# matthewygf/Tiresias

Measured on AMD Instinct MI355X. Metric: avg JCT + makespan on NSDI'19 Microsoft trace, 8×MI355X cluster, lower is better.
Workload: dtype bf16

## Files before the change

### csrc/bindings/ops.cpp

```cpp
#include <array>
#include <ATen/ATen.h>
#include <c10/hip/HIPStream.h>
#include <torch/library.h>

#include <functional>
#include <map>
#include <mutex>
#include <sstream>
#include <tuple>
#include <vector>

#include "tam/kernels.h"
#include "tam/launch.h"
#include "tam/gemm8p.h"

using at::Tensor;
using c10::optional;

namespace {

hipStream_t cur_stream(const Tensor& t) {
  return c10::hip::getCurrentHIPStream(t.device().index()).stream();
}

// ... 903 lines not shown
void avgpool_backward_op(const Tensor& dy, const Tensor& dx) {
  check_bf16(dy, "dy"); check_bf16(dx, "dx"); check_contig(dx, "dx");
  tam::avgpool_backward(bp(dy), bpm(dx), (int)dx.size(0), (int)(dx.size(1) * dx.size(2)),
                        (int)dx.size(3), cur_stream(dy));
}

void softmax_xent_op(const Tensor& logits, const Tensor& labels, const optional<Tensor>& dlogits,
                     const Tensor& loss_rows, double smoothing, double grad_scale,
                     int64_t ignore_index, int64_t tm_b) {
  check_bf16(logits, "logits"); check_contig(logits, "logits");
  TORCH_CHECK(labels.scalar_type() == at::kLong && labels.is_cuda() && labels.is_contiguous(),
              "tam.xent: labels contiguous int64 GPU");
  check_f32(loss_rows, "loss_rows");
  const int64_t V = logits.size(-1), rows = logits.numel() / V;
  TORCH_CHECK(labels.numel() == rows && loss_rows.numel() == rows, "tam.xent: row count");
  TORCH_CHECK(tm_b <= 0 || rows % tm_b == 0, "tam.xent: tm_b must divide the rows");
  tam::softmax_xent(bp(logits), labels.data_ptr<int64_t>(), opt_ptr<tam::bf16_t>(dlogits),
                    loss_rows.data_ptr<float>(), rows, (int)V, (float)smoothing, (float)grad_scale,
                    ignore_index, cur_stream(logits), tm_b);
}

void embedding_forward_op(const Tensor& table, const Tensor& ids, const Tensor& out, double scale, int64_t tm_b,
                          const optional<Tensor>& pos) {
  check_bf16(table, "table"); check_bf16(out, "out"); check_contig(table, "table");
  TORCH_CHECK(ids.scalar_type() == at::kLong && ids.is_contiguous(), "tam.embedding: ids");
  const int64_t D = table.size(1);
  TORCH_CHECK(D % 8 == 0, "tam.embedding: D % 8");
  TORCH_CHECK(out.numel() == ids.numel() * D, "tam.embedding: out size");
  TORCH_CHECK(tm_b <= 0 || ids.numel() % tm_b == 0, "tam.embedding: tm_b must divide the ids");
  const tam::bf16_t* pp = nullptr;
  int64_t prow = 0;
  if (pos.has_value() && pos->defined()) {
    check_bf16(*pos, "pos"); check_contig(*pos, "pos");
    TORCH_CHECK(pos->dim() == 2 && pos->size(1) == D, "tam.embedding: pos must be [S][D]");
    prow = pos->size(0);
    TORCH_CHECK(prow > 0 && (tm_b > 0 ? ids.numel() / tm_b == prow : ids.numel() % prow == 0),
                "tam.embedding: pos rows must equal the sequence length");
    pp = bp(*pos);
  }
  tam::embedding_forward(bp(table), ids.data_ptr<int64_t>(), bpm(out), ids.numel(), (int)D,
                         (float)scale, cur_stream(table), table.size(0), tm_b, pp, prow);
}
void embedding_backward_op(const Tensor& dout, const Tensor& ids, const Tensor& gtable, double scale, int64_t tm_b) {
  check_bf16(dout, "dout"); check_f32(gtable, "gtable"); check_contig(dout, "dout");
  TORCH_CHECK(ids.scalar_type() == at::kLong && ids.is_contiguous() && gtable.dim() == 2 &&
                  dout.numel() == ids.numel() * gtable.size(1), "tam.embedding_backward: shapes");
  TORCH_CHECK(tm_b <= 0 || ids.numel() % tm_b == 0, "tam.embedding_backward: tm_b must divide the ids");
  tam::embedding_backward(bp(dout), ids.data_ptr<int64_t>(), gtable.data_ptr<float>(), ids.numel(),
                          (int)gtable.size(1), (float)scale, cur_stream(dout), gtable.size(0), tm_b);
}

void conv_dma_policy_op(int64_t p) { tam::conv_dma_policy((int)p); }
void conv_halo_policy_op(int64_t p) { tam::conv_halo_policy((int)p); }
void colsum_policy_op(int64_t p) { tam::colsum_policy((int)p); }
void attn_short_policy_op(int64_t p) { tam::attn_short_policy((int)p); }
void conv_wgrad_c64_policy_op(int64_t p) { tam::conv_wgrad_c64_policy((int)p); }
void conv_wgrad_order_op(int64_t p) { tam::conv_wgrad_order((int)p); }
void conv_stem_policy_op(int64_t p) { tam::conv_stem_policy((int)p); }
void conv_wgrad_slab_policy_op(int64_t p) { tam::conv_wgrad_slab_policy((int)p); }
void conv_wgrad_force_op(int64_t bm, int64_t bn, int64_t splits, int64_t noatomic) {
  tam::conv_wgrad_force((int)bm, (int)bn, (int)splits, (int)noatomic);
}
int g_dma_policy = 1;
TAM_KNOB(g_dma_policy)
void gemm_dma_policy_op(int64_t p, int64_t cfg) {
  g_dma_policy = (int)p;
  tam::gemm_dma_policy(p == 2 ? 1 : 0, (int)cfg);
}

void gemm8p_policy_op(int64_t mode, int64_t tile) { tam::gemm8p_policy((int)mode, (int)tile); }
void gemm_pw_policy_op(int64_t on) { tam::gemm_pw_policy((int)on); }
void conv_pw_gemm_policy_op(int64_t mode, int64_t tile) { tam::conv_pw_gemm_policy((int)mode, (int)tile); }

std::string policy_names_op() {
  std::string out;
  for (const auto& k : tam::knob_registry()) {
    if (!out.empty()) out += ",";
    out += k.name;
  }
  return out;
}
std::vector<int64_t> policy_state_op() {
  std::vector<int64_t> v;
  for (const auto& k : tam::knob_registry()) v.push_back(*k.p);
  return v;
}
void policy_load_op(std::vector<int64_t> v) {
  auto& reg = tam::knob_registry();
  TORCH_CHECK(v.size() == reg.size(), "policy_load: ", v.size(), " values for ", reg.size(), " knobs");
  for (size_t i = 0; i < reg.size(); ++i) *reg[i].p = (int)v[i];
}
void gemm8p_group_op(int64_t g) { tam::gemm8p_group((int)g); }
void gemm8p_slab_force_op(int64_t sp) { tam::gemm8p_slab_force((int)sp); }
void gemm8p_sk_force_op(int64_t on) { g_sk_force = on != 0; }
void conv_split_policy_op(int64_t p) { tam::conv_split_policy((int)p); }
void optim_grid_op(int64_t b) { tam::optim_grid((int)b); }
void optim_variant_op(int64_t v) { tam::optim_variant((int)v); }
void gemm_skinny_policy_op(int64_t on, int64_t sp, int64_t nst) {
  tam::gemm_skinny_policy((int)on, (int)sp, (int)nst);
}

void gemm_force_op(int64_t cfg, int64_t splits) {
  tam::gemm_force((int)cfg, (int)splits);
  g_forced = cfg >= 0 || splits >= 1;
}

// ... 403 lines not shown
  m.def("conv_fwd(Tensor x, Tensor w, Tensor(a!) y, int stride, int pad, int dil, Tensor? bias, bool relu, Tensor(b!)? stats=None) -> int", &conv_fwd_op);
  m.def("conv_dgrad(Tensor dy, Tensor w, Tensor(a!) wt, Tensor(b!) dx, int stride, int pad, int dil, Tensor? mask) -> ()", &conv_dgrad_op);
  m.def("conv_weight_t_batch(Tensor[] w, Tensor(a!)[] wt) -> ()", &conv_weight_t_batch_op);
  m.def("gemm_wgrad_grouped(Tensor[] dy, Tensor[] x, Tensor(a!)[] dw, Tensor(b!)[] db, int[]? modes=None) -> ()", &gemm_wgrad_grouped_op);
  m.def("gemm_wgrad_grouped_ok(int M, int N, int K) -> bool", &gemm_wgrad_grouped_ok_op);
  m.def("gemm_grouped_tile(int tile) -> ()", &gemm_grouped_tile_op);
  m.def("conv_dgrad_pre(Tensor dy, Tensor w, Tensor wt, Tensor(a!) dx, int stride, int pad, int dil, Tensor? mask, Tensor(b!)? stats=None, Tensor? bnx=None, Tensor? bnmean=None, Tensor? bnrstd=None) -> int", &conv_dgrad_pre_op);
  m.def("conv_wgrad(Tensor dy, Tensor x, Tensor(a!) dw, int stride, int pad, int dil, int mode, Tensor(b!)? dbias=None, bool patch=True) -> ()", &conv_wgrad_op);
  m.def("conv_wgrad_deferred(Tensor dy, Tensor x, Tensor(a!) dw, int stride, int pad, int dil, int mode, Tensor(b!)? dbias, bool patch) -> (Tensor, int)", &conv_wgrad_deferred_op);
  m.def("wgrad_slab_reduce_many(Tensor[] slabs, int[] sp, Tensor(a!)[] dw, int[] mode) -> ()", &wgrad_slab_reduce_many_op);
  m.def("bn_forward(Tensor x, Tensor? res, Tensor(a!) y, Tensor gamma, Tensor beta, Tensor(b!)? run_mean, Tensor(c!)? run_var, Tensor(d!) save_mean, Tensor(e!) save_rstd, float eps, float momentum, bool relu, Tensor(f!)? sums=None, bool sums_ready=False, Tensor(g!)? ymask=None) -> ()", &bn_forward_op);
  m.def("bn_backward(Tensor dy, Tensor? y, Tensor x, Tensor mean, Tensor rstd, Tensor gamma, Tensor(a!) dx, Tensor(b!)? dres, Tensor(c!)? dgamma, Tensor(d!)? dbeta, bool relu, Tensor? addend=None, Tensor(e!)? sums=None, bool sums_ready=False, Tensor? ymask=None) -> ()", &bn_backward_op);
  m.def("ln_forward(Tensor x, Tensor g, Tensor b, Tensor(a!) y, Tensor(b!) mean, Tensor(c!) rstd, float eps, Tensor? addend=None, Tensor(d!)? sum_out=None, Tensor? drop_rec=None, int drop_site=0, int drop_thr=0, float drop_scale=1.0) -> ()", &ln_forward_op);
  m.def("ln_backward(Tensor dy, Tensor x, Tensor g, Tensor mean, Tensor rstd, Tensor(a!) dx, Tensor(b!) dg, Tensor(c!) db, Tensor? addend=None, Tensor(d!)? dr=None, Tensor? drop_rec=None, int drop_site=0, int drop_thr=0, float drop_scale=1.0) -> ()", &ln_backward_op);
  m.def("ln_backward_split(Tensor dy, Tensor x, Tensor g, Tensor mean, Tensor rstd, Tensor(a!) dx, Tensor(b!) ws, Tensor? addend=None, Tensor(c!)? dr=None, Tensor? drop_rec=None, int drop_site=0, int drop_thr=0, float drop_scale=1.0) -> int", &ln_backward_split_op);
  m.def("dropout_apply(Tensor x, Tensor(a!) y, Tensor rec, int site, int thr, float scale) -> ()", &dropout_apply_op);
  m.def("dropout_advance(Tensor(a!) rec) -> ()", &dropout_advance_op);
  m.def("col_reduce_acc(Tensor part, int nblk, int W, Tensor(a!) out0, Tensor(b!) out1, int split) -> ()", &col_reduce_acc_op);
  m.def("col_reduce_acc_batch(Tensor[] parts, int[] nblk, Tensor(a!)[] out0, Tensor(b!)[] out1) -> ()", &col_reduce_acc_batch_op);
  m.def("maxpool_forward(Tensor x, Tensor(a!) y, Tensor(b!) idx, int R, int S, int stride, int pad) -> ()", &maxpool_forward_op);
  m.def("maxpool_backward(Tensor dy, Tensor idx, Tensor(a!) dx, int R, int S, int stride, int pad) -> ()", &maxpool_backward_op);
  m.def("maxpool_k3s2_policy(int policy) -> ()", &maxpool_k3s2_policy_op);
  m.def("avgpool_forward(Tensor x, Tensor(a!) y) -> ()", &avgpool_forward_op);
  m.def("avgpool_backward(Tensor dy, Tensor(a!) dx) -> ()", &avgpool_backward_op);
  m.def("softmax_xent(Tensor logits, Tensor labels, Tensor(a!)? dlogits, Tensor(b!) loss_rows, float smoothing, float grad_scale, int ignore_index, int tm_b=0) -> ()", &softmax_xent_op);
  m.def("embedding_forward(Tensor table, Tensor ids, Tensor(a!) out, float scale, int tm_b=0, Tensor? pos=None) -> ()", &embedding_forward_op);
  m.def("embedding_backward(Tensor dout, Tensor ids, Tensor(a!) gtable, float scale, int tm_b=0) -> ()", &embedding_backward_op);
  m.def("sum_scale(Tensor x, Tensor(a!) out, float scale) -> ()", &sum_scale_op);
  m.def("rows_sum(Tensor[] outs, Tensor[] ins, int[] n_in) -> ()", &rows_sum_op);
  m.def("zero_(Tensor(a!) t) -> ()", &zero_op);
  m.def("colsum(Tensor x, Tensor(a!) out) -> ()", &colsum_op);
  m.def("gemm_force(int cfg, int splits) -> ()", &gemm_force_op);
  m.def("gemm8p_policy(int mode, int tile) -> ()", &gemm8p_policy_op);
  m.def("gemm_pw_policy(int on) -> ()", &gemm_pw_policy_op);
  m.def("conv_pw_gemm_policy(int mode, int tile) -> ()", &conv_pw_gemm_policy_op);
  m.def("policy_names() -> str", &policy_names_op);
  m.def("policy_state() -> int[]", &policy_state_op);
  m.def("policy_load(int[] v) -> ()", &policy_load_op);
  m.def("gemm8p_group(int g) -> ()", &gemm8p_group_op);
  m.def("gemm8p_slab_force(int sp) -> ()", &gemm8p_slab_force_op);
  m.def("gemm_skinny_policy(int on, int force_splits, int nst) -> ()", &gemm_skinny_policy_op);
  m.def("gemm8p_sk_force(int on) -> ()", &gemm8p_sk_force_op);
  m.def("conv_split_policy(int p) -> ()", &conv_split_policy_op);
  m.def("optim_variant(int v) -> ()", &optim_variant_op);
  m.def("optim_grid(int blocks) -> ()", &optim_grid_op);
  m.def("gemm_lib_policy(int policy) -> ()", &gemm_lib_policy_op);
  m.def("conv_dma_policy(int policy) -> ()", &conv_dma_policy_op);
  m.def("conv_wgrad_force(int bm, int bn, int splits, int noatomic=0) -> ()", &conv_wgrad_force_op);
  m.def("conv_wgrad_c64_policy(int policy) -> ()", &conv_wgrad_c64_policy_op);
  m.def("conv_wgrad_order(int flat) -> ()", &conv_wgrad_order_op);
  m.def("conv_stem_policy(int policy) -> ()", &conv_stem_policy_op);
  m.def("conv_wgrad_slab_policy(int policy) -> ()", &conv_wgrad_slab_policy_op);
  m.def("conv_halo_policy(int policy) -> ()", &conv_halo_policy_op);
  m.def("colsum_policy(int policy) -> ()", &colsum_policy_op);
  m.def("attn_short_policy(int policy) -> ()", &attn_short_policy_op);
  m.def("gemm_dma_policy(int policy, int cfg) -> ()", &gemm_dma_policy_op);
  m.def("gemm_routes() -> str", &gemm_routes_op);
  m.def("relu_backward(Tensor dy, Tensor y, Tensor(a!) dx) -> ()", &relu_backward_op);
  m.def("add(Tensor a, Tensor b, Tensor(a!) y) -> ()", &add_op);
  m.def("cast_f32_bf16(Tensor x, Tensor(a!) y) -> ()", &cast_op);
  m.def("sgd_step(Tensor(a!) w, Tensor(b!) g, Tensor(c!) mom, Tensor(d!) wb, float lr, float momentum, float wd, float gscale, bool nesterov, bool zero_grad, Tensor? guard=None, int zero_from=0, int wd_until=-1, Tensor? clip=None) -> ()", &sgd_op);
  m.def("adam_step(Tensor(a!) w, Tensor(b!) g, Tensor(c!) m, Tensor(d!) v, Tensor(e!) wb, float lr, float b1, float b2, float eps, float wd, int step, float gscale, bool zero_grad, Tensor? guard=None, int zero_from=0, int wd_until=-1, Tensor? clip=None) -> ()", &adam_op);
  m.def("sgd_step_bf16s(Tensor(a!) w, Tensor(b!) g, Tensor(c!) mom, Tensor(d!) wb, float lr, float momentum, float wd, float gscale, bool nesterov, bool zero_grad, int seed, int step, int base=0, Tensor? guard=None, int zero_from=0, int wd_until=-1, Tensor? clip=None) -> ()", &sgd_bf16s_op);
  m.def("adam_step_bf16s(Tensor(a!) w, Tensor(b!) g, Tensor(c!) m, Tensor(d!) v, Tensor(e!) wb, float lr, float b1, float b2, float eps, float wd, int step, float gscale, bool zero_grad, int seed, int base=0, Tensor? guard=None, int zero_from=0, int wd_until=-1, Tensor? clip=None) -> ()", &adam_bf16s_op);
  m.def("grad_sumsq(Tensor g, Tensor(a!) partials) -> ()", &grad_sumsq_op);
  m.def("grad_clip_finalize(Tensor partials, float max_norm, float gscale, Tensor(a!) clip) -> ()", &grad_clip_finalize_op);
  m.def("grad_sumsq_blocks(int n) -> int", &grad_sumsq_blocks_op);
  m.def("lars_step(Tensor(a!) w, Tensor(b!) g, Tensor(c!) mom, Tensor(d!) wb, float lr, float momentum, float wd, float eta, float gscale, Tensor tiles, Tensor seg_first, Tensor(e!) partials, Tensor(f!) ratios, Tensor? guard=None, int zero_from=0, int wd_until=-1, Tensor? clip=None) -> ()", &lars_op);
  m.def("lamb_step(Tensor(a!) w, Tensor(b!) g, Tensor(c!) m, Tensor(d!) v, Tensor(e!) wb, float lr, float b1, float b2, float eps, float wd, int step, float eta, float gscale, Tensor tiles, Tensor seg_first, Tensor(f!) partials, Tensor(g!) ratios, Tensor? guard=None, int zero_from=0, int wd_until=-1, Tensor? clip=None) -> ()", &lamb_op);
  m.def("trust_tile() -> int", &trust_tile_op);
  m.def("lstm_guard_step(Tensor(a!) err) -> ()", &lstm_guard_step_op);
  m.def("attn_forward(Tensor q, Tensor k, Tensor v, Tensor(a!) o, Tensor(b!) lse, bool causal, float scale, Tensor? kv_len, Tensor? drop_rec=None, int drop_site=0, int drop_thr=0, float drop_scale=1.0) -> ()", &attn_forward_op);
  m.def("attn_backward(Tensor q, Tensor k, Tensor v, Tensor o, Tensor dout, Tensor lse, Tensor(a!) dq, Tensor(b!) dk, Tensor(c!) dv, Tensor(d!) dq_acc, Tensor(e!) delta, bool causal, float scale, Tensor? kv_len, Tensor? drop_rec=None, int drop_site=0, int drop_thr=0, float drop_scale=1.0) -> ()", &attn_backward_op);
  m.def("lstm_step_forward(Tensor gx, Tensor w_hh, Tensor? h_prev, Tensor? c_prev, Tensor(a!) c_out, Tensor(b!) h_out, Tensor(c!) act) -> ()", &lstm_step_fwd_op);
  m.def("lstm_seq_forward(Tensor gx, Tensor w_hh, Tensor(a!) hs, Tensor(b!) cs, Tensor(c!) act, bool reverse, Tensor(d!) sync, Tensor(e!)? job_err=None, int grids=-1, int reserved_cus=0, bool zeroed=False) -> bool", &lstm_seq_fwd_op);
  m.def("lstm_seq_backward(Tensor act, Tensor cs, Tensor dH, Tensor w_hh, Tensor(a!) dG, bool reverse, Tensor(b!) sync, Tensor(c!)? job_err=None, int grids=-1, int reserved_cus=0, bool zeroed=False) -> bool", &lstm_seq_bwd_op);
  m.def("lstm_seq_policy(int ch) -> ()", &lstm_seq_policy_op);
  m.def("lstm_seq_shards(int ns) -> ()", &lstm_seq_shards_op);
  m.def("gemm_routes_load(str text) -> int", &gemm_routes_load_op);
  m.def("lstm_seq_residency(int grids, int reserved_cus) -> ()", &lstm_seq_residency_op);
  m.def("lstm_persist_timeouts(bool reset) -> int", &lstm_persist_timeouts_op);
  m.def("lstm_seq_spin_limit(int polls) -> ()", &lstm_seq_spin_limit_op);
  m.def("lstm_cell_forward(Tensor gates, Tensor? c_prev, Tensor(a!) c_out, Tensor(b!) h_out, Tensor(c!)? h_f32, Tensor(d!) act) -> ()", &lstm_fwd_op);
  m.def("lstm_cell_backward(Tensor act, Tensor? c_prev, Tensor? dh, Tensor? dc_next, Tensor(a!)? dgates, Tensor(b!)? dc_prev, Tensor(c!)? dgates_bf16) -> ()", &lstm_bwd_op);
}
```

### csrc/include/tam/conv_dma.h

```cpp
#pragma once
#include <cstdlib>
#include "tam/igemm.h"
#include "tam/slab.h"

namespace tam {

typedef __attribute__((address_space(3))) void cd_lds_void_t;

static __device__ __attribute__((aligned(256))) bf16_t g_cd_zero[128];

struct CDArgs {
  const bf16_t* src;
  const bf16_t* wgt;
  int M, Ng, Kd;
  int Hs, Ws, Cs;
  int P, Q;
  int stride, base_h, base_w;
  long ldb;
  int ntaps;
  int tap_dh[9], tap_dw[9], tap_kcol[9];
  int omap, oH, oW, osh, osw, ooh, oow;
  FastDiv fq, fp, fct;
};

// ... 121 lines not shown
    }
    if (stats) {
#pragma unroll
      for (int o = CPR; o < 64; o <<= 1)
#pragma unroll
        for (int e = 0; e < 8; ++e) {
          ssum[e] += __shfl_xor(ssum[e], o, 64);
          ssq[e] += __shfl_xor(ssq[e], o, 64);
        }
      float* red = (float*)(smem + W * 32 * LDW * 2);
      if (lane < CPR) {
#pragma unroll
        for (int e = 0; e < 8; ++e) {
          red[wid * 2 * WCOLS + lane * 8 + e] = ssum[e];
          red[wid * 2 * WCOLS + WCOLS + lane * 8 + e] = ssq[e];
        }
      }
      __syncthreads();
      if (wm == 0) {
        for (int e = lane; e < 2 * WCOLS; e += 64) {
          float t = 0.f;
#pragma unroll
          for (int k = 0; k < WM; ++k) t += red[(k + WM * wn) * 2 * WCOLS + e];
          unsafeAtomicAdd(ep.stats + (long)shard * 2 * Ng + (e < WCOLS ? cbase + e : Ng + cbase + (e - WCOLS)),
                          (double)t);
        }
      }
    }
    return;
  }

#pragma unroll
  for (int j = 0; j < TN; ++j) {
    const int col = n0 + wn * WCOLS + 16 * j + (lane & 15);
    if (col >= Ng) continue;
    const float bv = add_bias ? bf2f(ep.bias[col]) : 0.f;
#pragma unroll
    for (int i = 0; i < TM; ++i) {
#pragma unroll
      for (int r = 0; r < 4; ++r) {
        const long orow = rmap(wm * 64 + 16 * i + 4 * (lane >> 4) + r);
        if (orow < 0) continue;
        float v = acc[i][j][r] * ep.alpha + bv;
        if (ep.relu) v = fmaxf(v, 0.f);
        if (ep.mask && bf2f(ep.mask[orow * ep.ldm + col]) <= 0.f) v = 0.f;
        float* c = (float*)ep.c + orow * ep.ldc + col;
        if (ep.mode == 1) *c += v;
        else *c = v;
      }
    }
  }
}

template <int BN, int WN, int BM, int NST = 0>
__device__ __forceinline__ void conv_dma_body(const CDArgs& a, const Epi& ep, const int bid, const int kt_lo = 0,
                                              const int kt_hi = -1, float* __restrict__ slab = nullptr) {
  constexpr int WM = BM / 64;
  constexpr int W = WM * WN;
  constexpr int BK = 64;
  constexpr int A_BYTES = BM * BK * 2, B_BYTES = BN * BK * 2, STAGE = A_BYTES + B_BYTES;
  constexpr int STAGES = NST ? NST : (3 * STAGE <= 160 * 1024 ? 3 : 2);
  constexpr int AG = BM / 8 / W;
  constexpr int BG = BN / 8 / W;
  constexpr int D = AG + BG;
  constexpr int WCOLS = BN / WN;
  constexpr int TN = WCOLS / 16, TM = 4;
  __shared__ __attribute__((aligned(1024))) char smem[STAGES * STAGE];

  const int tid = threadIdx.x, lane = tid & 63, wid = tid >> 6;
  const int wm = wid % WM, wn = wid / WM;

  const int tiles_m = (a.M + BM - 1) / BM, tiles_n = (a.Ng + BN - 1) / BN;
  constexpr int GROUP = 8;
  const int per_group = GROUP * tiles_n;
  const int grp = bid / per_group;
  const int first_m = grp * GROUP;
  const int gsize = min(tiles_m - first_m, GROUP);
  const int tm = first_m + (bid % per_group) % gsize;
  const int tn = (bid % per_group) / gsize;
  const int m0 = tm * BM, n0 = tn * BN;

  const int lrow = lane >> 3;
  int abase[AG], ah[AG], aw[AG];
#pragma unroll
  for (int j = 0; j < AG; ++j) {
    const int rr = (wid + W * j) * 8 + lrow;
    const int c = (lane & 7) ^ ((rr >> 1) & 7);
    const int m = m0 + rr;
    if (m < a.M) {
      const int t = a.fq.div(m), q = m - t * a.Q, n = a.fp.div(t), p = t - n * a.P;
      const int hb = p * a.stride + a.base_h;
      const int wb = q * a.stride + a.base_w;
      ah[j] = hb;
      aw[j] = wb;
      abase[j] = ((n * a.Hs + hb) * a.Ws + wb) * a.Cs + c * 8;
    } else {
      ah[j] = -(1 << 28);
      aw[j] = 0;
      abase[j] = c * 8;
    }
  }
  const bf16_t* bptr[BG];
#pragma unroll
  for (int j = 0; j < BG; ++j) {
    const int rr = (wid + W * j) * 8 + lrow;
    const int c = (lane & 7) ^ ((rr >> 1) & 7);
    int n = n0 + rr;
    n = n < a.Ng ? n : a.Ng - 1;
    bptr[j] = a.wgt + (long)n * a.ldb + c * 8;
  }
  const int ctiles = a.Cs / BK;
  const int nk = (kt_hi < 0 ? a.Kd / BK : kt_hi) - kt_lo;

  auto issue = [&](int t, int st) {
    char* sa = smem + st * STAGE;
    char* sb = sa + A_BYTES;
    const int kt = kt_lo + t;
    const int tp = a.fct.div(kt), ct = kt - tp * ctiles;
    const int dh = a.tap_dh[tp], dw = a.tap_dw[tp];
    const int toff = (dh * a.Ws + dw) * a.Cs + ct * BK;
    const int kcol = a.tap_kcol[tp] + ct * BK;
#pragma unroll
    for (int j = 0; j < AG; ++j) {
// ... 17 lines not shown
#pragma unroll
    for (int j = 0; j < TN; ++j) acc[i][j] = f32x4_t{0.f, 0.f, 0.f, 0.f};

  if (nk > 0) {
#pragma unroll
    for (int t = 0; t < STAGES - 1; ++t)
      if (t < nk) issue(t, t);
    for (int t = 0; t < nk; ++t) {
      if constexpr (STAGES == 3) {
        if (t + 1 < nk) cd_vm_wait<D>();
        else cd_vm_wait<0>();
      } else {
        cd_vm_wait<0>();
      }
      cd_barrier();
      if (t + STAGES - 1 < nk) issue(t + STAGES - 1, (t + STAGES - 1) % STAGES);
      const int st = t % STAGES;
      const char* ta = smem + st * STAGE;
      const char* tb = ta + A_BYTES;
#pragma unroll
      for (int kk = 0; kk < BK / 32; ++kk) {
        s16x8_t fa[TM], fb[TN];
#pragma unroll
        for (int i = 0; i < TM; ++i) fa[i] = read_frag_k(ta, lane, wm * 64 + 16 * i, kk);
#pragma unroll
        for (int j = 0; j < TN; ++j) fb[j] = read_frag_k(tb, lane, wn * WCOLS + 16 * j, kk);
        __builtin_amdgcn_s_setprio(1);
#pragma unroll
        for (int i = 0; i < TM; ++i)
#pragma unroll
          for (int j = 0; j < TN; ++j)
            acc[i][j] = __builtin_amdgcn_mfma_f32_16x16x32_bf16(
                __builtin_bit_cast(bf16x8_t, fa[i]), __builtin_bit_cast(bf16x8_t, fb[j]), acc[i][j],
                0, 0, 0);
        __builtin_amdgcn_s_setprio(0);
      }
    }
  }

  if (slab) {
#pragma unroll
    for (int j = 0; j < TN; ++j) {
      const int col = n0 + wn * WCOLS + 16 * j + (lane & 15);
#pragma unroll
      for (int i = 0; i < TM; ++i)
#pragma unroll
        for (int r = 0; r < 4; ++r) {
          const int row = m0 + wm * 64 + 16 * i + 4 * (lane >> 4) + r;
          if (row < a.M) slab[(long)row * a.Ng + col] = acc[i][j][r];
        }
    }
    return;
  }
  cd_epilogue<BN, WN, BM>(acc, ep, smem, n0, a.Ng, tm % BN_SHARDS, [&](int lr) -> long {
    const int row = m0 + lr;
    return row < a.M ? cd_out_row(a, row) : -1L;
  });
}

template <int BN, int WN, int BM = 256, int NST = 0>
__global__ void __launch_bounds__(BM / 64 * 64 * WN, NST == 2 ? 2 : 1) conv_dma_split_kernel(CDArgs a, float* ws,
                                                                                            int kps) {
  const int nk = a.Kd / 64;
  const int lo = blockIdx.y * kps;
  conv_dma_body<BN, WN, BM, NST>(a, Epi{}, xcd_remap(blockIdx.x, gridDim.x), lo, min(nk, lo + kps),
                                 ws + (long)blockIdx.y * a.M * a.Ng);
}

static __global__ void __launch_bounds__(256) cd_slab_reduce_kernel(const float* __restrict__ ws, int sp, CDArgs a,
                                                             Epi ep, int rows_per_block) {
  __shared__ float red[2 * 2048];
  const int vs = a.Ng / 8, rpp = 256 / vs;
  const int cg = threadIdx.x % vs, rl = threadIdx.x / vs;
  const int c = cg * 8;
  float ssum[8], ssq[8];
#pragma unroll
  for (int e = 0; e < 8; ++e) ssum[e] = ssq[e] = 0.f;
  const long plane = (long)a.M * a.Ng;
  if (rl < rpp) {
    float bv[8];
#pragma unroll
    for (int e = 0; e < 8; ++e) bv[e] = ep.bias ? bf2f(ep.bias[c + e]) : 0.f;
    const int r0 = blockIdx.x * rows_per_block, r1 = min(a.M, r0 + rows_per_block);
    for (int m = r0 + rl; m < r1; m += rpp) {
      const float* src = ws + (long)m * a.Ng + c;
      float4 lo = *(const float4*)src, hi = *(const float4*)(src + 4);
      for (int z = 1; z < sp; ++z) {
        const float4 l2 = *(const float4*)(src + z * plane), h2 = *(const float4*)(src + z * plane + 4);
        lo.x += l2.x; lo.y += l2.y; lo.z += l2.z; lo.w += l2.w;
        hi.x += h2.x; hi.y += h2.y; hi.z += h2.z; hi.w += h2.w;
      }
      float v[8] = {lo.x, lo.y, lo.z, lo.w, hi.x, hi.y, hi.z, hi.w};
      const long orow = cd_out_row(a, m);
      bf16_t* dst = (bf16_t*)ep.c + orow * ep.ldc + c;
      uint4 mk = make_uint4(0u, 0u, 0u, 0u), old = make_uint4(0u, 0u, 0u, 0u);
      if (ep.mask) mk = *(const uint4*)(ep.mask + orow * ep.ldm + c);
      if (ep.mode == 1) old = *(const uint4*)dst;
      const uint32_t* mw = (const uint32_t*)&mk;
      const uint32_t* ow = (const uint32_t*)&old;
      uint32_t out[4];
#pragma unroll
      for (int e = 0; e < 8; ++e) {
        float t = v[e] * ep.alpha + bv[e];
        if (ep.relu) t = fmaxf(t, 0.f);
        if (ep.mask) {
          const uint32_t mb = (mw[e >> 1] >> (16 * (e & 1))) & 0xffffu;
          if ((mb & 0x8000u) || !(mb & 0x7fffu)) t = 0.f;
        }
        if (ep.mode == 1) t = bf2f(f2bf(t)) + bf2f((bf16_t)((ow[e >> 1] >> (16 * (e & 1))) & 0xffffu));
        v[e] = bf2f(f2bf(t));
      }
#pragma unroll
      for (int e = 0; e < 4; ++e) out[e] = pack_bf2(v[2 * e], v[2 * e + 1]);
      *(uint4*)dst = make_uint4(out[0], out[1], out[2], out[3]);
      if (ep.stats) {
#pragma unroll
        for (int e = 0; e < 8; ++e) { ssum[e] += v[e]; ssq[e] += v[e] * v[e]; }
      }
    }
  }
  if (!ep.stats) return;
  for (int e = threadIdx.x; e < 2 * a.Ng; e += 256) red[e] = 0.f;
  __syncthreads();
  if (rl < rpp) {
#pragma unroll
    for (int e = 0; e < 8; ++e) {
      atomicAdd(&red[c + e], ssum[e]);
      atomicAdd(&red[a.Ng + c + e], ssq[e]);
    }
  }
  __syncthreads();
  double* sh = ep.stats + (long)(blockIdx.x % BN_SHARDS) * 2 * a.Ng;
  for (int e = threadIdx.x; e < 2 * a.Ng; e += 256) unsafeAtomicAdd(sh + e, (double)red[e]);
}

template <int BN, int WN, int BM = 256, int NST = 0>
__global__ void __launch_bounds__(BM / 64 * 64 * WN, NST == 2 ? 2 : 1) conv_dma_kernel(CDArgs a, Epi ep) {
  conv_dma_body<BN, WN, BM, NST>(a, ep, xcd_remap(blockIdx.x, gridDim.x));
}

constexpr int CD_MULTI = 4;
struct CDMulti {
  CDArgs a[CD_MULTI];
  int t0[CD_MULTI + 1];
  int n;
};

template <int BN, int WN, int BM = 256>
__global__ void __launch_bounds__(BM / 64 * 64 * WN, 1) conv_dma_multi_kernel(CDMulti m, Epi ep) {
  const int bid = xcd_remap(blockIdx.x, gridDim.x);
  int c = 0;
  while (c + 1 < m.n && bid >= m.t0[c + 1]) ++c;
  conv_dma_body<BN, WN, BM>(m.a[c], ep, bid - m.t0[c]);
}

constexpr int CH_TR = 4, CH_TQ = 56;
constexpr int CH_PR = CH_TR + 2, CH_PW = CH_TQ + 2;
constexpr int CH_NP = CH_PR * CH_PW;
constexpr int CH_GROUPS = (CH_NP + 7) / 8;
constexpr int CH_PATCH = CH_GROUPS * 1024;
constexpr int CH_BSLOT = 64 * 64 * 2;

struct CHArgs {
  const bf16_t* src;
  const bf16_t* wgt;
  long ldb;
  int N, P, Q, Ng;
  int tap_oh[9], tap_ow[9], tap_kcol[9];
};

static __global__ void __launch_bounds__(256, 2) conv_halo_kernel(CHArgs a, Epi ep) {
  __shared__ __attribute__((aligned(1024))) char smem[CH_PATCH + 3 * CH_BSLOT];
  char* sp = smem;
  char* sb = smem + CH_PATCH;
  const int tid = threadIdx.x, lane = tid & 63, wid = tid >> 6;
  const int tiles_n = a.Ng / 64, tq = a.Q / CH_TQ, tp = a.P / CH_TR;
  const int bid = xcd_remap(blockIdx.x, gridDim.x);
  const int tn = bid % tiles_n;
  const int sidx = bid / tiles_n;
  const int q0 = (sidx % tq) * CH_TQ;
  const int p0 = ((sidx / tq) % tp) * CH_TR;
  const int n = sidx / (tq * tp);
  const int n0 = tn * 64;

#pragma unroll
  for (int j = 0; j < (CH_GROUPS + 3) / 4; ++j) {
    const int g = wid + 4 * j;
    if (g < CH_GROUPS) {
      const int i = 8 * g + (lane >> 3);
      const int pr = i / CH_PW, pc = i % CH_PW;
      const int h = p0 - 1 + pr, w = q0 - 1 + pc;
// ... 97 lines not shown
  };
  if (Ng % 256 == 0) consider(tm * (Ng / 256), 65536.0, 1.0, 256);
  if (Ng % 128 == 0) consider(tm * (Ng / 128), 32768.0, 0.92, 128);
  if (Ng % 128 == 0 && Kd >= 1024) consider(tm2 * (Ng / 128), 16384.0, 0.8, 128 | 0x1000);
  if (!pick && Ng % 64 == 0 && Kd >= 1024 && tm * (Ng / 64) >= 512) pick = 64;
  return pick;
}

struct CdSplit { int pick, sp; };
inline CdSplit cd_split_plan(const CDArgs& a, int pick0, int cus) {
  CdSplit best{pick0, 1};
  const int nk = a.Kd / 64;
  if (nk < 16) return best;
  double tbest = 1e30;
  const int codes[3] = {256, 128, 128 | 0x1000};
  const double eff[3] = {1.0, 0.92, 0.8};
  for (int c = 0; c < 3; ++c) {
    const int code = codes[c], bm = (code & 0x1000) ? 128 : 256, bn = code & 0xfff;
    if (a.Ng % bn) continue;
    if ((code & 0x1000) && a.Kd < 1024) continue;
    const long tiles = (long)((a.M + bm - 1) / bm) * (a.Ng / bn);
    const long slots = cus;
    for (int sp = 1; sp <= 8; ++sp) {
      if (sp > 1 && (nk / sp < 8 || (long)sp * a.M * a.Ng > (16L << 20))) break;
      const double block_us = 2.0 * bm * bn * (double)a.Kd / sp / (eff[c] * 2.4e6);
      const double waves = (double)((tiles * sp + slots - 1) / slots);
      double t = waves * block_us;
      if (sp > 1) t += (double)(sp + 1) * a.M * a.Ng * 4 / 4.0e6 + 3.0;
      if (t < tbest * 0.97) { tbest = t; best = CdSplit{code, sp}; }
    }
  }
  return best;
}

inline int cd_cus() {
  static int n = 0;
  if (!n) {
    int dev = 0;
    if (hipGetDevice(&dev) != hipSuccess ||
        hipDeviceGetAttribute(&n, hipDeviceAttributeMultiprocessorCount, dev) != hipSuccess || n < 1)
      n = 256;
  }
  return n;
}

inline bool cd_base_ok(const CDArgs& a, int force) {
  if (a.Cs % 64 != 0 || a.Kd % 64 != 0 || a.Kd < 64 || (a.Kd < 256 && !force)) return false;
  if (a.ntaps < 1 || a.ntaps > 9) return false;
  if ((long)a.Hs * a.Ws * a.Cs * ((a.M + a.P * a.Q - 1) / (a.P * a.Q)) >= (1L << 31)) return false;
  if ((long)a.Ng * a.ldb >= (1L << 31)) return false;
  return true;
}

inline long conv_dma_split_ws(const CDArgs& a, int force = 0) {
  if (!cd_base_ok(a, force)) return 0;
  const int pick = conv_dma_pick_bn(a.M, a.Ng, a.Kd, force);
  if (!pick || force || (a.Ng / 8) > 256) return 0;
  const CdSplit p = cd_split_plan(a, pick, cd_cus());
  return p.sp > 1 ? (long)p.sp * a.M * a.Ng : 0;
}

inline int launch_conv_dma(const CDArgs& a, const Epi& ep, hipStream_t s, int force = 0, float* ws = nullptr,
                           long ws_floats = 0) {
  if (!cd_base_ok(a, force)) return 0;
  const int pick = conv_dma_pick_bn(a.M, a.Ng, a.Kd, force);
  if (!pick) return 0;
  if (ws && !force && !ep.c_f32 && ep.mode != 2 && !ep.bnx && a.Ng / 8 <= 256) {
    const CdSplit p = cd_split_plan(a, pick, cd_cus());
    const int sp = p.sp;
    if (sp > 1 && (long)sp * a.M * a.Ng <= ws_floats) {
      const int nk = a.Kd / 64, kps = (nk + sp - 1) / sp, z = (nk + kps - 1) / kps;
      const bool t128 = (p.pick & 0x1000) != 0;
      const int bm = t128 ? 128 : 256, bn = p.pick & 0xfff;
      const dim3 grid((unsigned)(((a.M + bm - 1) / bm) * (a.Ng / bn)), (unsigned)z);
      if (t128) hipLaunchKernelGGL((conv_dma_split_kernel<128, 2, 128>), grid, dim3(256), 0, s, a, ws, kps);
      else if (bn == 256) hipLaunchKernelGGL((conv_dma_split_kernel<256, 2>), grid, dim3(512), 0, s, a, ws, kps);
      else if (bn == 128) hipLaunchKernelGGL((conv_dma_split_kernel<128, 2>), grid, dim3(512), 0, s, a, ws, kps);
      else hipLaunchKernelGGL((conv_dma_split_kernel<64, 1>), grid, dim3(256), 0, s, a, ws, kps);
      const int rpp = 256 / (a.Ng / 8);
      int rpb = (a.M + 511) / 512;
      rpb = (rpb + rpp - 1) / rpp * rpp;
      if (rpb < rpp) rpb = rpp;
      hipLaunchKernelGGL(cd_slab_reduce_kernel, dim3((unsigned)((a.M + rpb - 1) / rpb)), dim3(256), 0, s, ws, z,
                         a, ep, rpb);
      return bm;
    }
  }
  if (pick & 0x1000) {
    const int tiles = ((a.M + 127) / 128) * (a.Ng / 128);
    hipLaunchKernelGGL((conv_dma_kernel<128, 2, 128>), dim3(tiles), dim3(256), 0, s, a, ep);
    return 128;
  }
  const int bn = pick;
  const int tiles = ((a.M + 255) / 256) * (a.Ng / bn);
  switch (bn) {
    case 256:
      hipLaunchKernelGGL((conv_dma_kernel<256, 2>), dim3(tiles), dim3(512), 0, s, a, ep);
      break;
    case 128:
      hipLaunchKernelGGL((conv_dma_kernel<128, 2>), dim3(tiles), dim3(512), 0, s, a, ep);
      break;
    default:
      hipLaunchKernelGGL((conv_dma_kernel<64, 1>), dim3(tiles), dim3(256), 0, s, a, ep);
      break;
  }
  return 256;
}

inline bool launch_conv_dma_multi(const CDArgs* a, int n, const Epi& ep, hipStream_t s) {
  if (n < 1 || n > CD_MULTI) return false;
  const int Ng = a[0].Ng;
  for (int i = 0; i < n; ++i)
    if (a[i].Ng != Ng || a[i].Cs % 64 || a[i].Kd % 64 || a[i].ntaps < 1 || a[i].ntaps > 9) return false;
  struct Cand { int bm, bn; double eff; };
  const Cand cands[3] = {{256, 256, 1.0}, {256, 128, 0.92}, {128, 128, 0.8}};
  int pick = -1;
  double best = 1e30;
  for (int k = 0; k < 3; ++k) {
    if (Ng % cands[k].bn) continue;
// ... 513 lines not shown
```

### csrc/include/tam/launch.h

```cpp
#pragma once
#include <hip/hip_runtime.h>
#include "tam/igemm.h"

namespace tam {

void gemm_igemm(const bf16_t* A, long lda, bool a_kmajor, const bf16_t* B, long ldb, bool b_kmajor, int M,
                int N, int K, const Epi& ep, hipStream_t s);
void gemm(const bf16_t* A, long lda, bool a_kmajor, const bf16_t* B, long ldb, bool b_kmajor,
          int M, int N, int K, Epi ep, bool allow_split, hipStream_t s);
void gemm_select(const bf16_t* A, long lda, bool a_kmajor, const bf16_t* B, long ldb, bool b_kmajor,
                 int M, int N, int K, Epi ep, bool allow_split, hipStream_t s, int path);
void gemm_force(int cfg, int splits);
void gemm_dma_policy(int policy, int cfg);
void gemm8p_policy(int mode, int tile);
bool gemm_pw(const bf16_t* A, long lda, const bf16_t* B, long ldb, bf16_t* C, long ldc, long M, int N, int K,
             const bf16_t* mask, long ldm, double* stats, int relu, hipStream_t s);
bool gemm_pw_ok(long M, int N, int K, long lda, long ldb, long ldc);
void gemm_pw_policy(int on);
void gemm8p_group(int g);
int gemm8p_policy_mode();

struct GGProblem {
  const bf16_t* A;
  const bf16_t* B;
  float* C;
  float* bias;
  int M, N, K, lda, ldb;
  int mode = 1;
};
void gemm_wgrad_grouped(const GGProblem* probs, int n, hipStream_t s);
void wgrad_slab_reduce_many(const float* const* ws, const int* sp, const long* mn, float* const* dw,
                            const int* mode, int n, hipStream_t s);
bool gemm_wgrad_grouped_ok(int M, int N, int K, long lda, long ldb);
void gemm_grouped_tile(int t);

void gemm_slab_reduce(const float* ws, int sp, int M, int N, const Epi& ep, hipStream_t s);

bool gemm_skinny_ok(bool ak, bool bk, int M, int N, int K, long lda, long ldb);
int gemm_skinny_splits(int M, int N, int K);
void gemm_skinny(const bf16_t* A, long lda, const bf16_t* B, long ldb, bool bk, int M, int N, int K,
                 const Epi& ep, int sp, float* ws, hipStream_t s);
void gemm_skinny_policy(int on, int force_splits, int nst);

int conv_fwd(const bf16_t* x, const bf16_t* w, const ConvGeom& g, Epi ep, hipStream_t s, float* ws = nullptr,
             long ws_floats = 0, int pw_tile = -2);
long conv_fwd_split_ws(const ConvGeom& g, const Epi* ep = nullptr);
int conv_pw_gemm_kind(int M, int N, int K, const Epi& ep);
int conv_pw_route_get(int M, int N, int K, int kind);
struct ConvPwRoute {
  int M, N, K, kind, tile;
  float ms_conv, ms_p8;
};
void conv_pw_route_set(const ConvPwRoute& r, bool keep_existing);
int conv_pw_routes(ConvPwRoute* out, int cap);
void conv_pw_gemm_policy(int mode, int tile);
int conv_pw_gemm_mode();
bool conv_stem_fwd(const bf16_t* x, const bf16_t* w, const ConvGeom& g, const Epi& ep, hipStream_t s);
void conv_stem_policy(int p);
long conv_stem_wgrad_ws(const ConvGeom& g);
bool conv_stem_wgrad(const bf16_t* dy, const bf16_t* x, const ConvGeom& g, float* dw, int mode, float* ws,
                     long ws_floats, hipStream_t s);
long conv_dgrad_split_ws(const ConvGeom& g, const Epi* ep = nullptr);
void conv_split_policy(int p);
int conv_dgrad(const bf16_t* dy, const bf16_t* w, const bf16_t* wt, const ConvGeom& g, Epi ep,
               hipStream_t s, float* ws = nullptr, long ws_floats = 0, int pw_tile = -2);
int conv_wgrad(const bf16_t* dy, const bf16_t* x, const ConvGeom& g, Epi ep, hipStream_t s,
               float* dbias = nullptr, bool allow_patch = true, float* ws = nullptr, long ws_floats = 0,
               int* slab_defer = nullptr);
long conv_wgrad_split_ws(const ConvGeom& g);
void conv_wgrad_slab_policy(int p);
void conv_weight_t(const bf16_t* w, bf16_t* wt, const ConvGeom& g, hipStream_t s);
void conv_dma_policy(int p);
void conv_wgrad_force(int bm, int bn, int splits, int noatomic = 0);
void conv_wgrad_order(int flat);
void conv_wgrad_c64_policy(int p);
void conv_halo_policy(int p);
bool gemm_select_big_p8(bool ak, bool bk, int M, int N, int K, long lda, long ldb);

}
```

### csrc/kernels/conv.hip

```cpp
#include <cstdlib>
#include <map>
#include <mutex>
#include <tuple>

#include "tam/launch.h"
#include "tam/tiles.h"
#include "tam/conv_dma.h"
#include "tam/gemm8p.h"
#include "tam/kernels.h"

namespace tam {

static int g_conv_dma = 1;
TAM_KNOB(g_conv_dma)
void conv_dma_policy(int p) { g_conv_dma = p; }
static int g_conv_split = 1;
TAM_KNOB(g_conv_split)
void conv_split_policy(int p) { g_conv_split = p; }
static int g_conv_halo = [] {
  const char* e = getenv("TAM_CONV_HALO");
  return e ? atoi(e) : 1;
}();
TAM_KNOB(g_conv_halo)
void conv_halo_policy(int p) { g_conv_halo = p; }
static ::tam::KnobReg g_wgrad_force_knobs_[4] = {{"g_wgrad_force0", &g_wgrad_force[0]}, {"g_wgrad_force1", &g_wgrad_force[1]},
                                                  {"g_wgrad_force2", &g_wgrad_force[2]}, {"g_wgrad_force3", &g_wgrad_force[3]}};
void conv_wgrad_force(int bm, int bn, int splits, int noatomic) {
  g_wgrad_force[0] = bm; g_wgrad_force[1] = bn; g_wgrad_force[2] = splits; g_wgrad_force[3] = noatomic;
}

template <int BM, int BN>
static void fwd_tile(const bf16_t* x, const bf16_t* w, const ConvGeom& g, const Epi& ep, int sp,
                     hipStream_t s) {
  const int M = g.N * g.P * g.Q, Kd = g.R * g.S * g.C;
  LdConvFwdA<BM> la{x, g, M, Kd};
  la.with_divs();
  LdKMajor<BN> lb{w, Kd, g.K, Kd};
  launch_igemm<BM, BN>(la, lb, M, g.K, Kd, ep, sp, s);
}

static bool is_pointwise(const ConvGeom& g) {
  return g.R == 1 && g.S == 1 && g.stride == 1 && g.pad == 0;
}

static int g_conv_pw_gemm = [] {
  const char* e = getenv("TAM_CONV_PW_GEMM");
  return e ? atoi(e) : 1;
}();
static int g_conv_pw_gemm_tile = 0;
TAM_KNOB(g_conv_pw_gemm) TAM_KNOB(g_conv_pw_gemm_tile)
void conv_pw_gemm_policy(int mode, int tile) {
  g_conv_pw_gemm = mode;
  g_conv_pw_gemm_tile = tile;
}
int conv_pw_gemm_mode() { return g_conv_pw_gemm; }

static std::map<std::tuple<int, int, int, int>, ConvPwRoute> g_pw_routes;
static std::mutex g_pw_mu;

int conv_pw_gemm_kind(int M, int N, int K, const Epi& ep) {
  if (!g_conv_pw_gemm || ep.c_f32 || ep.mode != 0 || ep.bias || ep.alpha != 1.f || ep.bnx || ep.colsum_a) return -1;
  if (ep.mask && (ep.relu || ep.stats)) return -1;
  if (!gemm8p_ok(true, true, M, N, K, K, K) || gemm_pw_ok(M, N, K, K, K, ep.ldc)) return -1;
  if (N % 8 != 0 || (ep.ldc & 7) != 0 || (((uintptr_t)ep.c) & 15) != 0) return -1;
  if (ep.mask && ((ep.ldm & 7) != 0 || (((uintptr_t)ep.mask) & 15) != 0)) return -1;
  if (ep.mask) return 4;
  return (ep.stats ? 2 : 0) + (ep.relu ? 1 : 0);
}

int conv_pw_route_get(int M, int N, int K, int kind) {
  std::lock_guard<std::mutex> g(g_pw_mu);
  auto it = g_pw_routes.find({M, N, K, kind});
  return it == g_pw_routes.end() ? -1 : it->second.tile;
}

void conv_pw_route_set(const ConvPwRoute& r, bool keep_existing) {
  std::lock_guard<std::mutex> g(g_pw_mu);
// ... 289 lines not shown
```

Before: 0.1225.

## Add intra-block two-way K split for small-grid 3x3 DMA conv forward

Adds a conv_dma variant whose block holds two warp groups, each with its own LDS ring, splitting the K loop in half. The second group hands its partial accumulators to the first through LDS, and the first group runs the epilogue. It is used by default for 3x3 convolutions whose tile count is below the CU count but at least half of it, where the existing split planner would not split. The aim is more in-flight work per CU without a global workspace reduction. In exchange the block doubles its LDS and thread count and pays for a handoff barrier.

```diff
diff --git a/csrc/bindings/ops.cpp b/csrc/bindings/ops.cpp
--- a/csrc/bindings/ops.cpp
+++ b/csrc/bindings/ops.cpp
@@ -979,6 +979,8 @@
 
 void conv_dma_policy_op(int64_t p) { tam::conv_dma_policy((int)p); }
 void conv_halo_policy_op(int64_t p) { tam::conv_halo_policy((int)p); }
+void conv_ks2_policy_op(int64_t p) { tam::conv_ks2_policy((int)p); }
+int64_t conv_ks2_launches_op() { return tam::conv_ks2_launches(); }
 void colsum_policy_op(int64_t p) { tam::colsum_policy((int)p); }
 void attn_short_policy_op(int64_t p) { tam::attn_short_policy((int)p); }
 void conv_wgrad_c64_policy_op(int64_t p) { tam::conv_wgrad_c64_policy((int)p); }
@@ -1488,6 +1490,8 @@
   m.def("conv_stem_policy(int policy) -> ()", &conv_stem_policy_op);
   m.def("conv_wgrad_slab_policy(int policy) -> ()", &conv_wgrad_slab_policy_op);
   m.def("conv_halo_policy(int policy) -> ()", &conv_halo_policy_op);
+  m.def("conv_ks2_policy(int policy) -> ()", &conv_ks2_policy_op);
+  m.def("conv_ks2_launches() -> int", &conv_ks2_launches_op);
   m.def("colsum_policy(int policy) -> ()", &colsum_policy_op);
   m.def("attn_short_policy(int policy) -> ()", &attn_short_policy_op);
   m.def("gemm_dma_policy(int policy, int cfg) -> ()", &gemm_dma_policy_op);
diff --git a/csrc/include/tam/conv_dma.h b/csrc/include/tam/conv_dma.h
--- a/csrc/include/tam/conv_dma.h
+++ b/csrc/include/tam/conv_dma.h
@@ -197,9 +197,15 @@
   }
 }
 
-template <int BN, int WN, int BM, int NST = 0>
-__device__ __forceinline__ void conv_dma_body(const CDArgs& a, const Epi& ep, const int bid, const int kt_lo = 0,
-                                              const int kt_hi = -1, float* __restrict__ slab = nullptr) {
+__device__ __forceinline__ void cd_epilogue_idle(const Epi& ep) {
+  if (ep.c_f32) return;
+  cd_barrier();
+  if (ep.stats) __syncthreads();
+}
+
+template <int BN, int WN, int BM, int NST = 0, int KS = 1>
+__device__ __forceinline__ void conv_dma_body(const CDArgs& a, const Epi& ep, const int bid, int kt_lo = 0,
+                                              int kt_hi = -1, float* __restrict__ slab = nullptr) {
   constexpr int WM = BM / 64;
   constexpr int W = WM * WN;
   constexpr int BK = 64;
@@ -210,10 +216,20 @@
   constexpr int D = AG + BG;
   constexpr int WCOLS = BN / WN;
   constexpr int TN = WCOLS / 16, TM = 4;
-  __shared__ __attribute__((aligned(1024))) char smem[STAGES * STAGE];
-
-  const int tid = threadIdx.x, lane = tid & 63, wid = tid >> 6;
+  constexpr int RING = STAGES * STAGE;
+  static_assert(KS == 1 || KS == 2, "one K group, or two");
+  static_assert(KS * RING <= 160 * 1024, "the rings fit a CU's LDS");
+  __shared__ __attribute__((aligned(1024))) char smem_all[KS * RING];
+
+  const int kg = KS == 1 ? 0 : __builtin_amdgcn_readfirstlane((int)threadIdx.x / (W * 64));
+  const int tid = KS == 1 ? (int)threadIdx.x : (int)threadIdx.x % (W * 64), lane = tid & 63, wid = tid >> 6;
   const int wm = wid % WM, wn = wid / WM;
+  char* smem = smem_all + kg * RING;
+  if constexpr (KS > 1) {
+    const int part = a.Kd / BK / KS;
+    kt_lo = kg * part;
+    kt_hi = kt_lo + part;
+  }
 
   const int tiles_m = (a.M + BM - 1) / BM, tiles_n = (a.Ng + BN - 1) / BN;
   constexpr int GROUP = 8;
@@ -337,7 +353,31 @@
     }
     return;
   }
-  cd_epilogue<BN, WN, BM>(acc, ep, smem, n0, a.Ng, tm % BN_SHARDS, [&](int lr) -> long {
+  if constexpr (KS > 1) {
+    static_assert(W * TM * TN * 64 * 16 <= RING, "a partial tile fits one group's ring");
+    f32x4_t* hand = (f32x4_t*)(smem_all + RING);
+    cd_barrier();
+    if (kg == 1) {
+#pragma unroll
+      for (int i = 0; i < TM; ++i)
+#pragma unroll
+        for (int j = 0; j < TN; ++j) hand[((wid * TM + i) * TN + j) * 64 + lane] = acc[i][j];
+    }
+    cd_barrier();
+    if (kg == 1) {
+      cd_epilogue_idle(ep);
+      return;
+    }
+#pragma unroll
+    for (int i = 0; i < TM; ++i)
+#pragma unroll
+      for (int j = 0; j < TN; ++j) {
+        const f32x4_t o = hand[((wid * TM + i) * TN + j) * 64 + lane];
+#pragma unroll
+        for (int r = 0; r < 4; ++r) acc[i][j][r] += o[r];
+      }
+  }
+  cd_epilogue<BN, WN, BM>(acc, ep, smem_all, n0, a.Ng, tm % BN_SHARDS, [&](int lr) -> long {
     const int row = m0 + lr;
     return row < a.M ? cd_out_row(a, row) : -1L;
   });
@@ -422,6 +462,11 @@
 template <int BN, int WN, int BM = 256, int NST = 0>
 __global__ void __launch_bounds__(BM / 64 * 64 * WN, NST == 2 ? 2 : 1) conv_dma_kernel(CDArgs a, Epi ep) {
   conv_dma_body<BN, WN, BM, NST>(a, ep, xcd_remap(blockIdx.x, gridDim.x));
+}
+
+template <int BM, int WN, int BN>
+__global__ void __launch_bounds__(2 * (BM / 64) * 64 * WN, 1) conv_dma_ks2_kernel(CDArgs a, Epi ep) {
+  conv_dma_body<BN, WN, BM, 2, 2>(a, ep, xcd_remap(blockIdx.x, gridDim.x));
 }
 
 constexpr int CD_MULTI = 4;
@@ -625,10 +670,23 @@
   return true;
 }
 
+inline int g_conv_ks2 = 1;
+inline long g_conv_ks2_launches = 0;
+
+inline bool cd_ks2_ok(const CDArgs& a, int force) {
+  if (g_conv_ks2 <= 0 || force || a.ntaps != 9 || a.Ng % 128 != 0) return false;
+  const int nk = a.Kd / 64;
+  if ((nk & 1) || nk < 8) return false;
+  const long tiles = (long)((a.M + 127) / 128) * (a.Ng / 128);
+  if (tiles >= cd_cus()) return false;
+  if (g_conv_ks2 >= 2) return true;
+  return 2 * tiles >= cd_cus() && cd_split_plan(a, conv_dma_pick_bn(a.M, a.Ng, a.Kd, 0), cd_cus()).sp == 1;
+}
+
 inline long conv_dma_split_ws(const CDArgs& a, int force = 0) {
   if (!cd_base_ok(a, force)) return 0;
   const int pick = conv_dma_pick_bn(a.M, a.Ng, a.Kd, force);
-  if (!pick || force || (a.Ng / 8) > 256) return 0;
+  if (!pick || force || (a.Ng / 8) > 256 || cd_ks2_ok(a, force)) return 0;
   const CdSplit p = cd_split_plan(a, pick, cd_cus());
   return p.sp > 1 ? (long)p.sp * a.M * a.Ng : 0;
 }
@@ -638,6 +696,12 @@
   if (!cd_base_ok(a, force)) return 0;
   const int pick = conv_dma_pick_bn(a.M, a.Ng, a.Kd, force);
   if (!pick) return 0;
+  if (cd_ks2_ok(a, force)) {
+    const int tiles = ((a.M + 127) / 128) * (a.Ng / 128);
+    hipLaunchKernelGGL((conv_dma_ks2_kernel<128, 2, 128>), dim3(tiles), dim3(512), 0, s, a, ep);
+    ++g_conv_ks2_launches;
+    return 128;
+  }
   if (ws && !force && !ep.c_f32 && ep.mode != 2 && !ep.bnx && a.Ng / 8 <= 256) {
     const CdSplit p = cd_split_plan(a, pick, cd_cus());
     const int sp = p.sp;
diff --git a/csrc/include/tam/launch.h b/csrc/include/tam/launch.h
--- a/csrc/include/tam/launch.h
+++ b/csrc/include/tam/launch.h
@@ -75,6 +75,8 @@
 void conv_wgrad_order(int flat);
 void conv_wgrad_c64_policy(int p);
 void conv_halo_policy(int p);
+void conv_ks2_policy(int p);
+long conv_ks2_launches();
 bool gemm_select_big_p8(bool ak, bool bk, int M, int N, int K, long lda, long ldb);
 
 }
diff --git a/csrc/kernels/conv.hip b/csrc/kernels/conv.hip
--- a/csrc/kernels/conv.hip
+++ b/csrc/kernels/conv.hip
@@ -23,6 +23,13 @@
 }();
 TAM_KNOB(g_conv_halo)
 void conv_halo_policy(int p) { g_conv_halo = p; }
+static const int g_conv_ks2_env_ = [] {
+  const char* e = getenv("TAM_CONV_KS2");
+  return g_conv_ks2 = e ? atoi(e) : 1;
+}();
+TAM_KNOB(g_conv_ks2)
+void conv_ks2_policy(int p) { g_conv_ks2 = p; }
+long conv_ks2_launches() { return g_conv_ks2_launches; }
 static ::tam::KnobReg g_wgrad_force_knobs_[4] = {{"g_wgrad_force0", &g_wgrad_force[0]}, {"g_wgrad_force1", &g_wgrad_force[1]},
                                                   {"g_wgrad_force2", &g_wgrad_force[2]}, {"g_wgrad_force3", &g_wgrad_force[3]}};
 void conv_wgrad_force(int bm, int bn, int splits, int noatomic) {
```

Measured after the change: 0.1229. Within noise of the previous version (+0.3%).
